# autonomousvision/LaRa

Hardware: AMD Instinct MI355X
Metric: novel-view frames/sec @512x512 (4-view in, 2DGS fwd+bwd) (higher is better)
Workload: dtype f32 raster + bf16-MFMA/f32-accumulate encoder (+ bf16-autocast coarse decoder MLP, as the reference's bf16-mixed)

## Files before the change

### lara_amd/csrc/composite.hip

```cpp
#include "common.h"
#include "wave.h"

namespace {

constexpr int FWD_CHUNK = 512;
constexpr int REC4 = 6;

__device__ __forceinline__ void cross3(const float a[3], const float b[3], float o[3]) {
    o[0] = a[1] * b[2] - a[2] * b[1];
    o[1] = a[2] * b[0] - a[0] * b[2];
    o[2] = a[0] * b[1] - a[1] * b[0];
}

template <int CHUNK>
__device__ __forceinline__ uint32_t stage_entry(const float4 *__restrict__ geom, const uint32_t id,
                                                const float4 cb, const bool valid, const float X0,
                                                const float Y0, float4 *rec, uint32_t *ids,
                                                const int e = threadIdx.x, uint2 *mask_out = nullptr) {
    float4 r0 = make_float4(0.f, 0.f, 0.f, 0.f), r1 = r0, r2 = r0, r3 = r0, r4 = r0, r5 = r0;
    uint32_t mask_lo = 0, mask_hi = 0, rectpack = 0;
    int gx0 = 0, gx1 = -1, gy0 = 0, gy1 = -1;
    if (valid) {
        gx0 = (int)ceilf(fminf(fmaxf((cb.x - X0 - 1.f) * 0.5f, 0.f), 8.f));
        gx1 = (int)floorf(fminf(fmaxf((cb.y - X0) * 0.5f, -1.f), 7.f));
        gy0 = (int)ceilf(fminf(fmaxf((cb.z - Y0 - 1.f) * 0.5f, 0.f), 8.f));
        gy1 = (int)floorf(fminf(fmaxf((cb.w - Y0) * 0.5f, -1.f), 7.f));
    }
    if (gx0 <= gx1 && gy0 <= gy1) {
        const float4 *g = geom + (size_t)id * 5;
        const float4 g0 = g[0], g1 = g[1], g2 = g[2], g3 = g[3], g4 = g[4];
        const float Tu[3] = {g0.x, g0.y, g0.z}, Tv[3] = {g0.w, g1.x, g1.y}, Tw[3] = {g1.z, g1.w, g2.x};
        const float k0[3] = {X0 * Tw[0] - Tu[0], X0 * Tw[1] - Tu[1], X0 * Tw[2] - Tu[2]};
        const float l0[3] = {Y0 * Tw[0] - Tv[0], Y0 * Tw[1] - Tv[1], Y0 * Tw[2] - Tv[2]};
        float A[3], B[3], C[3];
        cross3(k0, l0, A);
        cross3(Tw, l0, B);
        cross3(k0, Tw, C);
        const float cx = g2.y - X0, cy = g2.z - Y0, opa = g2.w;
        const float tau = 2.0f * __logf(255.0f * opa) * 1.001f + 0.01f;
        const float nb = B[0] * B[0] + B[1] * B[1], qa = nb - tau * B[2] * B[2];
        const bool ellipse = qa > 1e-5f * (nb + tau * B[2] * B[2]);
        const float inv_qa = ellipse ? __builtin_amdgcn_rcpf(qa) : 0.f;
        const float bx0 = (float)(2 * gx0), bx1 = (float)(2 * gx1 + 1);
        uint32_t colsum = 0;
        for (int by = gy0; by <= gy1; by++) {
            float lo = 1e9f, hi = -1e9f;
#pragma unroll
            for (int q = 0; q < 2; q++) {
                const float y = (float)(2 * by + q);
                const float u0 = A[0] + y * C[0], u1 = A[1] + y * C[1], u2 = A[2] + y * C[2];
                const float qb = u0 * B[0] + u1 * B[1] - tau * (u2 * B[2]);
                const float qc = u0 * u0 + u1 * u1 - tau * (u2 * u2);
                const float disc = qb * qb - qa * qc + 4e-6f * (qb * qb);
                if (!ellipse) {
                    lo = bx0; hi = bx1;
                } else if (disc >= 0.f) {
                    const float sq = __builtin_amdgcn_sqrtf(disc);
                    lo = fminf(lo, (-qb - sq) * inv_qa);
                    hi = fmaxf(hi, (-qb + sq) * inv_qa);
                }
                const float h = 0.5f * tau - (y - cy) * (y - cy);
                if (h >= 0.f) {
                    const float sh = __builtin_amdgcn_sqrtf(h);
                    lo = fminf(lo, cx - sh);
                    hi = fmaxf(hi, cx + sh);
                }
            }
            const int ilo = (int)ceilf(fmaxf(lo - 0.02f, bx0)), ihi = (int)floorf(fminf(hi + 0.02f, bx1));
            if (ilo <= ihi) {
                const uint32_t cols = ((2u << (ihi >> 1)) - 1u) & ~((1u << (ilo >> 1)) - 1u);
                colsum |= cols;
                if (by < 4) mask_lo |= cols << (8 * by);
                else mask_hi |= cols << (8 * (by - 4));
            }
        }
        if (colsum) {
            const int rx0 = __builtin_ctz(colsum), rx1 = 31 - __builtin_clz(colsum);
            const int ry0 = mask_lo ? (__builtin_ctz(mask_lo) >> 3) : 4 + (__builtin_ctz(mask_hi) >> 3);
            const int ry1 = mask_hi ? 4 + ((31 - __builtin_clz(mask_hi)) >> 3) : ((31 - __builtin_clz(mask_lo)) >> 3);
            rectpack = (uint32_t)rx0 | ((uint32_t)rx1 << 4) | ((uint32_t)ry0 << 8) | ((uint32_t)ry1 << 12) | (1u << 16);
            r0 = make_float4(A[0], A[1], A[2], B[0]);
            r1 = make_float4(B[1], B[2], C[0], C[1]);
            r2 = make_float4(C[2], cx, cy, Tw[0]);
            r3 = make_float4(Tw[1], Tw[2], opa, __uint_as_float(mask_lo));
            r4 = make_float4(g3.x, g3.y, g3.z, g4.x);
            r5 = make_float4(g4.y, g4.z, __uint_as_float(mask_hi), 0.f);
        }
    }
    rec[0 * CHUNK + e] = r0; rec[1 * CHUNK + e] = r1; rec[2 * CHUNK + e] = r2;
    rec[3 * CHUNK + e] = r3; rec[4 * CHUNK + e] = r4; rec[5 * CHUNK + e] = r5;
    if (ids) ids[e] = valid ? id : 0u;
    if (mask_out && valid) *mask_out = make_uint2(mask_lo, mask_hi);
    return rectpack;
}

template <int CHUNK>
__device__ __forceinline__ void stage_entry_masked(const float4 *__restrict__ geom, const uint32_t id, const uint2 mask,
                                                   const bool valid, const float X0, const float Y0, float4 *rec,
                                                   uint32_t *ids, const int e) {
    float4 r0 = make_float4(0.f, 0.f, 0.f, 0.f), r1 = r0, r2 = r0, r3 = r0, r4 = r0, r5 = r0;
    if (valid && (mask.x | mask.y)) {
        const float4 *g = geom + (size_t)id * 5;
        const float4 g0 = g[0], g1 = g[1], g2 = g[2], g3 = g[3], g4 = g[4];
        const float Tu[3] = {g0.x, g0.y, g0.z}, Tv[3] = {g0.w, g1.x, g1.y}, Tw[3] = {g1.z, g1.w, g2.x};
        const float k0[3] = {X0 * Tw[0] - Tu[0], X0 * Tw[1] - Tu[1], X0 * Tw[2] - Tu[2]};
        const float l0[3] = {Y0 * Tw[0] - Tv[0], Y0 * Tw[1] - Tv[1], Y0 * Tw[2] - Tv[2]};
        float A[3], B[3], C[3];
        cross3(k0, l0, A);
        cross3(Tw, l0, B);
        cross3(k0, Tw, C);
        r0 = make_float4(A[0], A[1], A[2], B[0]);
        r1 = make_float4(B[1], B[2], C[0], C[1]);
        r2 = make_float4(C[2], g2.y - X0, g2.z - Y0, Tw[0]);
        r3 = make_float4(Tw[1], Tw[2], g2.w, __uint_as_float(mask.x));
        r4 = make_float4(g3.x, g3.y, g3.z, g4.x);
        r5 = make_float4(g4.y, g4.z, __uint_as_float(mask.y), 0.f);
    }
    rec[0 * CHUNK + e] = r0; rec[1 * CHUNK + e] = r1; rec[2 * CHUNK + e] = r2;
    rec[3 * CHUNK + e] = r3; rec[4 * CHUNK + e] = r4; rec[5 * CHUNK + e] = r5;
    ids[e] = valid ? id : 0u;
}

struct Hit {
    float sx, sy, rz, depth, G, alpha, ddx, ddy;
    bool use3d;
};

struct EntryRec { float4 r0, r1, r2, r3; };
template <int CHUNK>
__device__ __forceinline__ EntryRec load_entry(const float4 *rec, const int j) {
    EntryRec e;
    e.r0 = rec[0 * CHUNK + j]; e.r1 = rec[1 * CHUNK + j]; e.r2 = rec[2 * CHUNK + j]; e.r3 = rec[3 * CHUNK + j];
    return e;
}

__device__ __forceinline__ bool eval_rec(const EntryRec &e, const float lx, const float ly, Hit &h,
                                         float Tw[3], float &opa) {
    const float4 r0 = e.r0, r1 = e.r1, r2 = e.r2, r3 = e.r3;
    const float px = r0.x + lx * r0.w + ly * r1.z;
    const float py = r0.y + lx * r1.x + ly * r1.w;
    const float pz = r0.z + lx * r1.y + ly * r2.x;
    Tw[0] = r2.w; Tw[1] = r3.x; Tw[2] = r3.y; opa = r3.z;
    h.rz = __builtin_amdgcn_rcpf(pz);
    h.sx = px * h.rz; h.sy = py * h.rz;
    const float rho3d = h.sx * h.sx + h.sy * h.sy;
    h.ddx = r2.y - lx; h.ddy = r2.z - ly;
    const float rho2d = FILTER_INV_SQUARE * (h.ddx * h.ddx + h.ddy * h.ddy);
    h.use3d = rho3d <= rho2d;
    const float rho = fminf(rho3d, rho2d);
    h.depth = h.use3d ? (h.sx * Tw[0] + h.sy * Tw[1]) + Tw[2] : Tw[2];
    const float power = -0.5f * rho;
    h.G = __expf(power);
    h.alpha = fminf(0.99f, opa * h.G);
    return (pz != 0.0f) & (h.depth >= NEAR_N) & !(power > 0.0f) & !(h.alpha < 1.0f / 255.0f);
}

__device__ __forceinline__ unsigned long long quad_masks(const uint32_t bm, const int qx4, const int grp) {
    unsigned long long m = 0ull;
#pragma unroll
    for (int g = 0; g < 16; g++) {
        const int bit = (g >> 2) * 8 + qx4 + (g & 3);
        const unsigned long long b = __ballot((bm >> bit) & 1u);
        m = (grp == g) ? b : m;
    }
    return m;
}

struct FwdPixel {
    float T = 1.0f, C0 = 0.f, C1 = 0.f, C2 = 0.f, N0 = 0.f, N1 = 0.f, N2 = 0.f;
    float Dd = 0.f, M1 = 0.f, M2 = 0.f, distortion = 0.f, median_depth = 0.f;
    uint32_t last_contributor = 0, median_contributor = 0;
    bool done = false;

    template <int CHUNK>
    __device__ __forceinline__ void blend(const float4 *rec, const int j, const int base, bool valid,
                                          const Hit &h) {
        valid = valid && !done;
        const float test_T = T * (1.0f - h.alpha);
        const bool kill = valid && test_T < 0.0001f;
        done = done || kill;
        valid = valid && !kill;
        if (__ballot(valid) == 0ull) return;
        const float4 r4 = rec[4 * CHUNK + j], r5 = rec[5 * CHUNK + j];
        const float a = valid ? h.alpha : 0.f;
        const float depth = valid ? h.depth : 1.0f;
        const float w = a * T;
        const float A = 1.0f - T;
        const float mm = FAR_N / (FAR_N - NEAR_N) * (1.0f - NEAR_N * __builtin_amdgcn_rcpf(depth));
        distortion += (mm * mm * A + M2 - 2.0f * mm * M1) * w;
        Dd += depth * w;
        M1 += mm * w;
        M2 += mm * mm * w;
        const bool med = valid && T > 0.5f;
        median_depth = med ? depth : median_depth;
        median_contributor = med ? (uint32_t)(base + j + 1) : median_contributor;
        N0 += r4.x * w; N1 += r4.y * w; N2 += r4.z * w;
        C0 += r4.w * w; C1 += r5.x * w; C2 += r5.y * w;
        T = valid ? test_T : T;
        last_contributor = valid ? (uint32_t)(base + j + 1) : last_contributor;
    }

};

template <bool KEEP>
__global__ void __launch_bounds__(256)
composite_fwd_kernel(ViewDev v, const uint32_t *__restrict__ header, const uint2 *__restrict__ ranges,
                     const uint32_t *__restrict__ point_list, const float4 *__restrict__ geom,
                     const uint32_t *__restrict__ tile_order, const float4 *__restrict__ cullbox,
                     float *__restrict__ final_T, uint32_t *__restrict__ n_contrib,
                     const uint32_t *__restrict__ seg_base, const uint32_t *__restrict__ seg_cnt,
                     float *__restrict__ ckpt, uint2 *__restrict__ pair_mask, uint32_t *__restrict__ tile_maxc,
                     uint32_t *__restrict__ seg_cost,
                     float *__restrict__ out_color, float *__restrict__ out_allmap, const ViewBatch vb) {
    {
        const long long sst = vb.state_stride, HWb = (long long)v.H * v.W * 4;
        header = l2d_view_ptr(header, sst); ranges = l2d_view_ptr(ranges, sst); point_list = l2d_view_ptr(point_list, sst);
        geom = l2d_view_ptr(geom, sst); tile_order = l2d_view_ptr(tile_order, sst); cullbox = l2d_view_ptr(cullbox, sst);
        final_T = l2d_view_ptr(final_T, sst); n_contrib = l2d_view_ptr(n_contrib, sst); seg_base = l2d_view_ptr(seg_base, sst);
        seg_cnt = l2d_view_ptr(seg_cnt, sst); ckpt = l2d_view_ptr(ckpt, sst); pair_mask = l2d_view_ptr(pair_mask, sst);
        tile_maxc = l2d_view_ptr(tile_maxc, sst); seg_cost = l2d_view_ptr(seg_cost, sst);
        out_color = l2d_view_ptr(out_color, 3 * HWb); out_allmap = l2d_view_ptr(out_allmap, 7 * HWb);
        v.bg = vb.bg[blockIdx.z];
    }
    constexpr int CHUNK = FWD_CHUNK;
    static_assert(L2D_SEG % FWD_CHUNK == 0, "segment boundaries must fall on round boundaries");
    __shared__ float4 rec[REC4 * CHUNK];
    __shared__ unsigned long long qmask[4][16][CHUNK / 64];
    uint32_t &s_cost = *(uint32_t *)&rec[5 * CHUNK + 0].w;
    uint32_t &s_tmax = *(uint32_t *)&rec[5 * CHUNK + 1].w;
    uint32_t &s_ndone = *(uint32_t *)&rec[5 * CHUNK + 2].w;
    const int tile = (v.dbg & 8u) ? (int)blockIdx.x : (int)tile_order[blockIdx.x];
    const int tx = tile % v.gx, ty = tile / v.gx;
    const int wave = threadIdx.x >> 6, lane = threadIdx.x & 63;
    const int grp = lane >> 2;
    const int lxi = (wave & 1) * 8 + (grp & 3) * 2 + (lane & 1);
    const int lyi = (wave >> 1) * 8 + (grp >> 2) * 2 + ((lane >> 1) & 1);
    const int pxi = tx * TILE + lxi, pyi = ty * TILE + lyi;
    const bool inside = pxi < v.W && pyi < v.H;
    const size_t HW = (size_t)v.H * v.W;
    const size_t pix = (size_t)pyi * v.W + pxi;
    const float lx = (float)lxi, ly = (float)lyi;
    const float X0 = (float)(tx * TILE), Y0 = (float)(ty * TILE);

    if (header[1]) {
        if (inside) {
            const float qnan = __uint_as_float(0x7fc00000u);
            for (int ch = 0; ch < 3; ch++) out_color[ch * HW + pix] = qnan;
            for (int ch = 0; ch < 7; ch++) out_allmap[ch * HW + pix] = qnan;
            if (KEEP) {
                for (int ch = 0; ch < L2D_CKPT_F; ch++) final_T[pix + ch * HW] = qnan;
                n_contrib[pix] = 0; n_contrib[pix + HW] = 0;
            }
        }
        return;
    }

    const uint2 range = ranges[tile];
    const int total = (int)(range.y - range.x);
    const int lo = 0, hi = total;
    FwdPixel px;
    px.done = !inside;
    uint32_t *dbg_hdr = const_cast<uint32_t *>(header);
    const long long dbg_t0 = (v.dbg & 32u) ? (long long)__builtin_readcyclecounter() : 0ll;
    int dbg_rounds = 0;

    const int tid = threadIdx.x;
    const uint32_t cost_nb = KEEP ? seg_cnt[tile] : 0u;
    uint32_t *const cost_full = KEEP ? seg_cost + seg_base[tile] : nullptr,
             *const cost_last = KEEP ? seg_cost + (v.cap / L2D_SEG + 1u) + tile : nullptr;
    if (KEEP)
        for (uint32_t q = tid; q <= cost_nb; q += 256) *(q < cost_nb ? cost_full + q : cost_last) = 0u;
    int cost_round = -1;
    constexpr int SPT = CHUNK / 256;
    uint32_t id1[SPT], id2[SPT];
    float4 cb1[SPT];
#pragma unroll
    for (int q = 0; q < SPT; q++) {
        const int o = lo + q * 256 + tid;
        id1[q] = o < hi ? point_list[range.x + o] : 0u;
        id2[q] = CHUNK + o < hi ? point_list[range.x + CHUNK + o] : 0u;
    }
#pragma unroll
    for (int q = 0; q < SPT; q++) cb1[q] = lo + q * 256 + tid < hi ? cullbox[id1[q]] : make_float4(0.f, 0.f, 0.f, 0.f);
    if (threadIdx.x < 3) *(uint32_t *)&rec[5 * CHUNK + threadIdx.x].w = 0u;
    __syncthreads();
    for (int base = lo; base < hi; base += CHUNK) {
        {
            const bool wave_done = __ballot(px.done) == ~0ull;
            if (wave_done && lane == 0) atomicAdd(&s_ndone, 1u);
            __syncthreads();
            if (s_ndone == 4u) break;
        }
        if (KEEP && tid == 0) {
            if (cost_round >= 0) { if ((uint32_t)cost_round < cost_nb) cost_full[cost_round] = s_cost; else *cost_last += s_cost; }
            s_cost = 0u;
        }
        cost_round = (base - lo) / CHUNK;
        dbg_rounds++;
        if (KEEP && base && base % L2D_SEG == 0 && !px.done) {
            float *ck = ckpt + ((size_t)seg_base[tile] + (size_t)(base / L2D_SEG - 1)) * (L2D_CKPT_F * 256) + tid;
            ck[0 * 256] = px.T; ck[1 * 256] = px.M1; ck[2 * 256] = px.M2;
            ck[3 * 256] = px.C0; ck[4 * 256] = px.C1; ck[5 * 256] = px.C2;
            ck[6 * 256] = px.Dd; ck[7 * 256] = px.N0; ck[8 * 256] = px.N1; ck[9 * 256] = px.N2;
        }
#pragma unroll
        for (int q = 0; q < SPT; q++) {
            const int o = q * 256 + tid;
            const uint32_t id0 = id1[q];
            const float4 cb0 = cb1[q];
            id1[q] = id2[q];
            id2[q] = base + 2 * CHUNK + o < hi ? point_list[range.x + base + 2 * CHUNK + o] : 0u;
            cb1[q] = base + CHUNK + o < hi ? cullbox[id1[q]] : make_float4(0.f, 0.f, 0.f, 0.f);
            stage_entry<CHUNK>(geom, id0, cb0, base + o < hi, X0, Y0, rec, nullptr, o,
                               KEEP && base + o < hi ? pair_mask + range.x + base + o : nullptr);
        }
        __syncthreads();
        if (__ballot(!px.done) == 0ull) continue;
        const int nw = (min(CHUNK, hi - base) + 63) >> 6;
        unsigned long long *qm = &qmask[wave][grp][0];
#pragma unroll 1
        for (int w = 0; w < nw; w++) {
            const float4 *mrec = rec + ((wave >> 1) ? 5 : 3) * CHUNK + w * 64 + lane;
            const uint32_t bm = __float_as_uint((wave >> 1) ? mrec->z : mrec->w);
            unsigned long long m = 0ull;
            if (__ballot((bm & (0x0f0f0f0fu << ((wave & 1) * 4))) != 0u) != 0ull) m = quad_masks(bm, (wave & 1) * 4, grp);
            if ((lane & 3) == 0) qm[w] = m;
        }
        int w = 0;
        unsigned long long mm = qm[0];
        if (((__ballot(px.done) >> (lane & ~3)) & 0xfull) == 0xfull) { mm = 0ull; w = nw; }
        auto next = [&](bool &has, int &j) {
            while (mm == 0ull && w + 1 < nw) { w++; mm = qm[w]; }
            has = mm != 0ull;
            j = has ? 64 * w + __builtin_ctzll(mm) : 0;
            mm &= mm - 1ull;
        };
        bool hA0, hA1, hB0 = false, hB1 = false;
        int jA0, jA1, jB0 = 0, jB1 = 0;
        next(hA0, jA0);
        next(hA1, jA1);
        EntryRec rA0 = load_entry<CHUNK>(rec, jA0), rA1 = load_entry<CHUNK>(rec, jA1), rB0, rB1;
        auto trip = [&](const EntryRec &c0, const EntryRec &c1, const int j0, const int j1, const bool has0, const bool has1,
                        EntryRec &x0, EntryRec &x1, int &k0, int &k1, bool &n0, bool &n1) {
            next(n0, k0);
            next(n1, k1);
            x0 = load_entry<CHUNK>(rec, k0);
            x1 = load_entry<CHUNK>(rec, k1);
            Hit h0, h1;
            float Tw0[3], Tw1[3], opa0, opa1;
            const bool e0 = eval_rec(c0, lx, ly, h0, Tw0, opa0) && has0;
            const bool e1 = eval_rec(c1, lx, ly, h1, Tw1, opa1) && has1;
            if (v.dbg & 4u) {
                atomicAdd(&dbg_hdr[4], ((lane & 3) == 0) ? (unsigned)has0 + (unsigned)has1 : 0u);
                atomicAdd(&dbg_hdr[5], (unsigned)e0 + (unsigned)e1);
                if (lane == 0) atomicAdd(&dbg_hdr[6], 1u);
            }
            px.blend<CHUNK>(rec, j0, base, e0, h0);
            px.blend<CHUNK>(rec, j1, base, e1, h1);
            if (((__ballot(px.done) >> (lane & ~3)) & 0xfull) == 0xfull) { mm = 0ull; w = nw; n0 = false; n1 = false; }
        };
        uint32_t ntrips = 0;
        while (true) {
            if (__ballot(hA0) == 0ull) break;
            trip(rA0, rA1, jA0, jA1, hA0, hA1, rB0, rB1, jB0, jB1, hB0, hB1);
            ntrips++;
            if (__ballot(hB0) == 0ull) break;
            trip(rB0, rB1, jB0, jB1, hB0, hB1, rA0, rA1, jA0, jA1, hA0, hA1);
            ntrips++;
        }
        if (KEEP && lane == 0 && ntrips) atomicAdd(&s_cost, ntrips);
    }
    const float T = px.T;
    if (KEEP) {
        if (threadIdx.x == 0) s_tmax = 0u;
        __syncthreads();
        uint32_t m = px.last_contributor;
#pragma unroll
        for (int d = 1; d < 64; d <<= 1) m = max(m, (uint32_t)__shfl_xor((int)m, d, 64));
        if (lane == 0) atomicMax(&s_tmax, m);
        __syncthreads();
        if (threadIdx.x == 0) {
            tile_maxc[tile] = s_tmax;
            if (cost_round >= 0) { if ((uint32_t)cost_round < cost_nb) cost_full[cost_round] = s_cost; else *cost_last += s_cost; }
        }
    }
// ... 49 lines not shown
#pragma unroll
    for (int c = 0; c < 3; c++) {
        float d = dp[c];
        asm volatile("" : "+v"(d));
        const float t = d + dpp_move<0xB1, 0xf>(d);
        const float tq = q[c] + dpp_move<0xB1, 0xf>(q[c]);
        const float mine = k.a1 * t + (k.a2 * d + k.a3 * tq);
        const float send = k.b1 * t + (k.b2 * d + k.b3 * tq);
        r[c] = mine + dpp_move<0x4E, 0xf>(send);
    }
    float v1[5];
#pragma unroll
    for (int i = 0; i < 5; i++) {
        const float mine = b0 ? h[2 * i + 1] : h[2 * i];
        const float send = b0 ? h[2 * i] : h[2 * i + 1];
        v1[i] = mine + dpp_move<0xB1, 0xf>(send);
    }
#pragma unroll
    for (int i = 0; i < 2; i++) {
        const float mine = b1 ? v1[2 * i + 1] : v1[2 * i];
        const float send = b1 ? v1[2 * i] : v1[2 * i + 1];
        r[3 + i] = mine + dpp_move<0x4E, 0xf>(send);
    }
    r[5] = v1[4] + dpp_move<0x4E, 0xf>(v1[4]);
}
__device__ __forceinline__ void quad_reduce_scatter16(const float dp[3], const float q[3], const float h[4], const QuadCoef &k,
                                                      float r[4], const int lane) {
    const bool b0 = lane & 1, b1 = lane & 2;
#pragma unroll
    for (int c = 0; c < 3; c++) {
        float d = dp[c], qq = q[c];
        asm volatile("" : "+v"(d));
        asm volatile("" : "+v"(qq));
        const float t = d + dpp_move<0xB1, 0xf>(d);
        const float tq = qq + dpp_move<0xB1, 0xf>(qq);
        const float mine = k.a1 * t + (k.a2 * d + k.a3 * tq);
        const float send = k.b1 * t + (k.b2 * d + k.b3 * tq);
        r[c] = mine + dpp_move<0x4E, 0xf>(send);
    }
    float v1[2];
#pragma unroll
    for (int i = 0; i < 2; i++) {
        const float mine = b0 ? h[2 * i + 1] : h[2 * i];
        const float send = b0 ? h[2 * i] : h[2 * i + 1];
        v1[i] = mine + dpp_move<0xB1, 0xf>(send);
    }
    const float mine = b1 ? v1[1] : v1[0];
    const float send = b1 ? v1[0] : v1[1];
    r[3] = mine + dpp_move<0x4E, 0xf>(send);
}

constexpr int SLAB_WIN = 128;
constexpr int SLAB_CHUNK = 128;
constexpr int SLAB_POOL = 374;
constexpr int SLAB_F = 24;
constexpr int SLAB_F_COLOR = 16;
constexpr int SLAB_POOL_COLOR = SLAB_POOL * SLAB_F / SLAB_F_COLOR;

template <bool MAPS>
__global__ void __launch_bounds__(256)
composite_bwd_kernel(ViewDev v, const uint32_t *__restrict__ header, const uint2 *__restrict__ ranges,
                     const uint32_t *__restrict__ point_list, const float4 *__restrict__ geom,
                     const uint32_t *__restrict__ tile_order, const float4 *__restrict__ cullbox,
                     const float *__restrict__ final_T, const uint32_t *__restrict__ n_contrib,
                     const uint32_t *__restrict__ seg_base, const uint32_t *__restrict__ seg_cnt,
                     const uint32_t *__restrict__ bwd_order,
                     const uint2 *__restrict__ bwd_items, const float *__restrict__ ckpt,
                     const uint2 *__restrict__ pair_mask, const uint32_t *__restrict__ tile_maxc,
                     const float *__restrict__ dL_dcolor, const float *__restrict__ dL_dallmap,
                     const uint32_t *__restrict__ pair_pos,
                     float4 *__restrict__ pair_grad, uint8_t *__restrict__ pair_valid, const ViewBatch vb) {
    {
        const long long sst = vb.state_stride, qst = vb.scratch_stride, HWb = (long long)v.H * v.W * 4;
        header = l2d_view_ptr(header, sst); ranges = l2d_view_ptr(ranges, sst); point_list = l2d_view_ptr(point_list, sst);
        geom = l2d_view_ptr(geom, sst); tile_order = l2d_view_ptr(tile_order, sst); cullbox = l2d_view_ptr(cullbox, sst);
        final_T = l2d_view_ptr(final_T, sst); n_contrib = l2d_view_ptr(n_contrib, sst); seg_base = l2d_view_ptr(seg_base, sst);
        seg_cnt = l2d_view_ptr(seg_cnt, sst); bwd_order = l2d_view_ptr(bwd_order, sst); bwd_items = l2d_view_ptr(bwd_items, sst);
        ckpt = l2d_view_ptr(ckpt, sst); pair_mask = l2d_view_ptr(pair_mask, sst); pair_pos = l2d_view_ptr(pair_pos, sst);
        tile_maxc = l2d_view_ptr(tile_maxc, sst);
        pair_grad = l2d_view_ptr(pair_grad, qst); pair_valid = l2d_view_ptr(pair_valid, qst);
        dL_dcolor = l2d_view_ptr(dL_dcolor, 3 * HWb); dL_dallmap = l2d_view_ptr(dL_dallmap, 7 * HWb);
        v.bg = vb.bg[blockIdx.z];
    }
    constexpr int WIN = SLAB_WIN;
    constexpr int POOL = MAPS ? SLAB_POOL : SLAB_POOL_COLOR, SF = MAPS ? SLAB_F : SLAB_F_COLOR;
    __shared__ float4 rec[REC4 * WIN];
    __shared__ __attribute__((aligned(16))) float pool[(POOL + 1) * SF];
    __shared__ uint16_t s_base_[2][SLAB_CHUNK];
    __shared__ unsigned long long s_live_[2][SLAB_CHUNK];
    __shared__ uint32_t s_ql[64];
    __shared__ uint32_t s_id_[2][WIN];
    __shared__ uint2 s_mask[WIN];
    __shared__ int s_nfit_[2];
    __shared__ uint32_t s_total_[2];
    if (header[1]) return;
    const unsigned long long dbg_t0 = (v.dbg & 32u) ? wall_clock64() : 0ull;
    int dbg_rounds = 0;
    uint32_t dbg_windows = 0, dbg_trips = 0, dbg_entries = 0, dbg_slots = 0, dbg_rows = 0;
    unsigned long long dbg_tp = 0ull;
    uint32_t dbg_ph[5] = {0u, 0u, 0u, 0u, 0u};
#define DBG_PHASE(k) do { if (v.dbg & 64u) { const unsigned long long t__ = __builtin_readcyclecounter(); dbg_ph[k] += (uint32_t)(t__ - dbg_tp); dbg_tp = t__; } } while (0)
    if (v.dbg & 64u) dbg_tp = __builtin_readcyclecounter();
    const uint32_t n_full = header[3];
    int tile, seg;
    if (header[22]) {
        if (blockIdx.x >= n_full + (uint32_t)v.tiles) return;
        const uint2 it = bwd_items[blockIdx.x];
        tile = (int)it.x; seg = (int)it.y;
    } else if (blockIdx.x < n_full) {
        const uint2 it = bwd_items[blockIdx.x];
        tile = (int)it.x; seg = (int)it.y;
    } else if (blockIdx.x - n_full < (uint32_t)v.tiles) {
        tile = (int)bwd_order[blockIdx.x - n_full];
        seg = (int)seg_cnt[tile];
    } else {
        return;
    }
    const uint2 range = ranges[tile];
    const int seg_lo = seg * L2D_SEG;
    const int seg_hi = seg == (int)seg_cnt[tile] ? (int)(range.y - range.x) : seg_lo + L2D_SEG;
    const int total = min((int)tile_maxc[tile], seg_hi);
    const int lo = seg_lo;
    if (total <= lo) return;
    const int tx = tile % v.gx, ty = tile / v.gx;
    const int tid = threadIdx.x, wave = tid >> 6, lane = tid & 63;
    const int grp = lane >> 2;
    const int lxi = (wave & 1) * 8 + (grp & 3) * 2 + (lane & 1);
    const int lyi = (wave >> 1) * 8 + (grp >> 2) * 2 + ((lane >> 1) & 1);
    const int pxi = tx * TILE + lxi, pyi = ty * TILE + lyi;
    const bool inside = pxi < v.W && pyi < v.H;
    const size_t HW = (size_t)v.H * v.W;
    const size_t pix = inside ? (size_t)pyi * v.W + pxi : 0;
    const float lx = (float)lxi, ly = (float)lyi;
    const float X0 = (float)(tx * TILE), Y0 = (float)(ty * TILE);

    const float T_final = inside ? final_T[pix] : 0.f;
    float T = T_final;
    const uint32_t last_contributor = inside ? n_contrib[pix] : 0u;
    const uint32_t median_contributor = (MAPS && inside) ? n_contrib[pix + HW] : 0u;
    float dpix[3] = {0.f, 0.f, 0.f}, dnrm[3] = {0.f, 0.f, 0.f};
    float dL_ddepth = 0.f, dL_daccum = 0.f, dL_dmedian = 0.f, dL_dreg = 0.f;
    float final_D = 0.f, final_D2 = 0.f;
    if (inside) {
        for (int ch = 0; ch < 3; ch++) dpix[ch] = dL_dcolor[ch * HW + pix];
        if constexpr (MAPS) {
            dL_ddepth = dL_dallmap[0 * HW + pix];
            dL_daccum = dL_dallmap[1 * HW + pix];
// ... 58 lines not shown
                    volatile unsigned long long *vlive = live_;
                    vlive[2 * lane] = 0ull;
                    vlive[2 * lane + 1] = 0ull;
                    if (jm < SLAB_CHUNK) atomicOr(&live_[jm], 1ull << lane);
                    __builtin_amdgcn_wave_barrier();
                    la = vlive[2 * lane];
                    lb = la | vlive[2 * lane + 1];
                    unsigned long long ex = lb;
#pragma unroll
                    for (int d = 1; d < 64; d <<= 1) {
                        const uint32_t ylo = __shfl_up((uint32_t)ex, d, 64), yhi = __shfl_up((uint32_t)(ex >> 32), d, 64);
                        if (lane >= d) ex |= ((unsigned long long)yhi << 32) | ylo;
                    }
                    const uint32_t plo = __shfl_up((uint32_t)ex, 1, 64), phi = __shfl_up((uint32_t)(ex >> 32), 1, 64);
                    const unsigned long long before = lane ? (((unsigned long long)phi << 32) | plo) : 0ull;
                    la |= before; lb |= before;
                }
                uint32_t c[2];
#pragma unroll
                for (int q = 0; q < 2; q++) {
                    const int slot = s0_ + 2 * lane + q;
                    unsigned long long mk = 0ull;
                    if (slot < wcnt_) {
                        const uint2 mw = side ? s_mask[slot] : make_uint2(__float_as_uint(rec[3 * WIN + slot].w), __float_as_uint(rec[5 * WIN + slot].z));
                        mk = (((unsigned long long)mw.y << 32) | mw.x) & (q ? lb : la);
                    }
                    live_[2 * lane + q] = mk;
                    c[q] = (uint32_t)__builtin_popcountll(mk);
                }
                uint32_t incl = c[0] + c[1];
#pragma unroll
                for (int d = 1; d < 64; d <<= 1) {
                    const uint32_t y = __shfl_up(incl, d, 64);
                    if (lane >= d) incl += y;
                }
                const uint32_t b0 = incl - c[0] - c[1], b1 = incl - c[1];
                const unsigned long long f0 = __ballot(s0_ + 2 * lane < wcnt_ && b1 <= (uint32_t)POOL);
                const unsigned long long f1 = __ballot(s0_ + 2 * lane + 1 < wcnt_ && incl <= (uint32_t)POOL);
                const int L = f1 == ~0ull ? 64 : __builtin_ctzll(~f1);
                if (lane == 0) s_nfit_[buf] = L == 64 ? 128 : 2 * L + (int)((f0 >> L) & 1ull);
                base_[2 * lane] = (uint16_t)b0;
                base_[2 * lane + 1] = (uint16_t)b1;
                if (lane == 63) s_total_[buf] = incl;
    };
    {
        const int wcnt = min(WIN, total - lo);
        if (stager) {
            const uint32_t id0 = total - 1 - se >= lo ? point_list[range.x + total - 1 - se] : 0u;
            const uint2 mk0 = total - 1 - se >= lo ? pair_mask[range.x + total - 1 - se] : make_uint2(0u, 0u);
            id1 = total - WIN - 1 - se >= lo ? point_list[range.x + total - WIN - 1 - se] : 0u;
            mk1 = total - WIN - 1 - se >= lo ? pair_mask[range.x + total - WIN - 1 - se] : make_uint2(0u, 0u);
            id2 = total - 2 * WIN - 1 - se >= lo ? point_list[range.x + total - 2 * WIN - 1 - se] : 0u;
            mk2 = total - 2 * WIN - 1 - se >= lo ? pair_mask[range.x + total - 2 * WIN - 1 - se] : make_uint2(0u, 0u);
            stage_entry_masked<WIN>(geom, id0, mk0, se < wcnt, X0, Y0, rec, s_id_[0], se);
        }
        __syncthreads();
        if (wave == 3) size_round(total, wcnt, 0, 0, false);
        __syncthreads();
        DBG_PHASE(0);
    }
    int cur = 0, wb = 0;
    for (int whi = total; whi > lo; whi -= WIN) {
        const int wcnt = min(WIN, whi - lo);
        const bool more_windows = whi - WIN > lo;
        dbg_windows++;
        if (stager) s_mask[se] = mk1;
        unsigned long long wm0 = 0ull, wm1 = 0ull;

        for (int s0 = 0; s0 < wcnt;) {
            dbg_rounds++;
            const unsigned long long *const s_live = s_live_[cur];
            const uint16_t *const s_base = s_base_[cur];
            const uint32_t *const s_id = s_id_[wb];
            const int nfit = s_nfit_[cur];
            if (v.dbg & 512u) { dbg_entries += (uint32_t)nfit; dbg_slots += nfit < SLAB_CHUNK ? (uint32_t)s_base[nfit] : min(s_total_[cur], (uint32_t)POOL); }

            {
                if (s0 == 0) {
#pragma unroll
                    for (int k = 0; k < 2; k++) {
                        const float4 *mrec = rec + ((wave >> 1) ? 5 : 3) * WIN + 64 * k + lane;
                        const uint32_t bm = __float_as_uint((wave >> 1) ? mrec->z : mrec->w);
                        unsigned long long m = 0ull;
                        if (__ballot((bm & (0x0f0f0f0fu << ((wave & 1) * 4))) != 0u) != 0ull) m = quad_masks(bm, (wave & 1) * 4, grp);
                        if (k == 0) wm0 = m; else wm1 = m;
                    }
                }
                unsigned long long m0 = wm0, m1 = wm1;
                {
                    int sh = s0;
                    if (sh >= 64) { m0 = m1; m1 = 0ull; sh -= 64; }
                    if (sh) { m0 = (m0 >> sh) | (m1 << (64 - sh)); m1 >>= sh; }
                    if (nfit < 64) { m0 &= (1ull << nfit) - 1ull; m1 = 0ull; }
                    else if (nfit < 128) m1 &= (1ull << (nfit - 64)) - 1ull;
                }
                const int jmin = whi - s0 - (int)quad_last;
                if (jmin > 0) {
                    m0 = jmin >= 64 ? 0ull : m0 & (~0ull << jmin);
                    m1 = jmin >= 128 ? 0ull : (jmin > 64 ? m1 & (~0ull << (jmin - 64)) : m1);
                }
                uint32_t mm = (uint32_t)m0, q1 = (uint32_t)(m0 >> 32), q2 = (uint32_t)m1, q3 = (uint32_t)(m1 >> 32);
                int jb = 0;
                auto trip = [&]() __attribute__((always_inline)) {
                    dbg_trips++;
                    while (mm == 0u && (q1 | q2 | q3) != 0u) { mm = q1; q1 = q2; q2 = q3; q3 = 0u; jb += 32; }
                    const bool has = mm != 0u;
                    const int j = jb + (has ? __builtin_ctz(mm) : 0);
                    mm &= mm - 1u;
                    const int ws = s0 + j;
                    const uint32_t contributor = (uint32_t)(whi - 1 - ws);
                    const EntryRec ent = load_entry<WIN>(rec, ws);
                    Hit h;
                    float Tw[3], opa;
                    const bool active = eval_rec(ent, lx, ly, h, Tw, opa) && has && contributor < last_contributor;
                    const float4 r4 = rec[4 * WIN + ws], r5 = rec[5 * WIN + ws];
                    const float nrm[3] = {r4.x, r4.y, r4.z}, rgb[3] = {r4.w, r5.x, r5.y};
                    if constexpr (!MAPS) {
                        (void)nrm;
                        const float alpha = active ? h.alpha : 0.f;
                        const float inv_1ma = __builtin_amdgcn_rcpf(1.f - alpha);
                        const float T_new = T * inv_1ma;
                        const float w = alpha * T_new;
                        const float gval = __builtin_fmaf(rgb[2], dpix[2], __builtin_fmaf(rgb[0], dpix[0], rgb[1] * dpix[1]));
                        const float accum_new = mul_legacy(last_alpha, last_g) + (1.f - last_alpha) * accum_g;
                        float dL_dalpha = gval - accum_new;
                        dL_dalpha = __builtin_fmaf(T_new, dL_dalpha, -((T_final * inv_1ma) * bg_dot_dpixel));
                        T = T_new;
                        accum_g = accum_new;
                        last_g = gval;
                        last_alpha = alpha;
                        const float da = active ? dL_dalpha : 0.f;
                        const float sx = h.sx, sy = h.sy;
                        const float rz3 = (active && h.use3d) ? h.rz : 0.f;
                        const float qG = opa * da * h.G;
                        const float dL_dsx = -mul_legacy(qG, sx), dL_dsy = -mul_legacy(qG, sy);
                        const float dpx = dL_dsx * rz3, dpy = dL_dsy * rz3;
                        const float dpv[3] = {dpx, dpy, -(mul_legacy(dpx, sx) + mul_legacy(dpy, sy))};
                        const float qG2 = h.use3d ? 0.f : -FILTER_INV_SQUARE * qG;
                        const float q3[3] = {h.G * da, qG2 * h.ddx, qG2 * h.ddy};
                        const float h4[4] = {w * dpix[0], w * dpix[1], w * dpix[2], w};
// ... 23 lines not shown
                    const float dL_dweight = (final_D2 + m_d * m_d * final_A - 2.f * m_d * final_D) * dL_dreg;
                    dL_dalpha += dL_dweight - last_dL_dT;
                    const float dLdT_new = mul_legacy(alpha, dL_dweight) + (1.f - alpha) * last_dL_dT;
                    const float dL_dmd = 2.0f * (T_new * alpha) * (m_d * final_A - final_D) * dL_dreg;
                    dL_dz += dL_dmd * dmd_dd;
                    dL_dalpha *= T_new;
                    dL_dalpha += (-T_final * inv_1ma) * bg_dot_dpixel;
                    dL_dz += w * dL_ddepth;
                    T = T_new;
                    accum_g = accum_new;
                    last_g = gval;
                    last_alpha = alpha;
                    last_dL_dT = dLdT_new;
                    const float ww = w, da = active ? dL_dalpha : 0.f, dz = active ? dL_dz : 0.f;
                    const float sx = h.sx, sy = h.sy;
                    const float rz3 = (active && h.use3d) ? h.rz : 0.f;
                    const float qv[3] = {mul_legacy(dz, sx), mul_legacy(dz, sy), dz};
                    const float qG = opa * da * h.G;
                    const float dL_dsx = dz * Tw[0] - mul_legacy(qG, sx);
                    const float dL_dsy = dz * Tw[1] - mul_legacy(qG, sy);
                    const float dpx = dL_dsx * rz3, dpy = dL_dsy * rz3;
                    const float dpv[3] = {dpx, dpy, -(mul_legacy(dpx, sx) + mul_legacy(dpy, sy))};
                    const float qG2 = h.use3d ? 0.f : -FILTER_INV_SQUARE * qG;
                    const float hv[10] = {qG2 * h.ddx, qG2 * h.ddy, ww * dnrm[0], ww * dnrm[1], ww * dnrm[2], h.G * da,
                                          ww * dpix[0], ww * dpix[1], ww * dpix[2], ww};
                    float r[6];
                    quad_reduce_scatter(dpv, qv, hv, qcoef, r, lane);
#pragma unroll
                    for (int i = 0; i < 6; i++) asm volatile("" : "+v"(r[i]));
                    const unsigned long long lv = s_live[has ? j : 0];
                    const int rank = __builtin_popcount((uint32_t)lv & below_lo) + __builtin_popcount((uint32_t)(lv >> 32) & below_hi);
                    float *ps = pool + ((int)s_base[has ? j : 0] + rank) * SLAB_F + (lane & 3);
                    if (has) {
                        ps[0] = r[0]; ps[4] = r[1]; ps[8] = r[2]; ps[12] = r[3]; ps[16] = r[4];
                        if (!(lane & 2)) ps[20] = r[5];
                    }
                    }
                };
                while (__ballot((mm | q1 | q2 | q3) != 0u) != 0ull) {
                    trip();
                    if (__ballot((mm | q1 | q2 | q3) != 0u) == 0ull) break;
                    trip();
                }
            }
            __syncthreads();
            DBG_PHASE(3);

            if ((wave << 5) < nfit && !(v.dbg & 2u)) {
                const int e = tid >> 1, part = tid & 1;
                const int ws = min(s0 + e, WIN - 1);
                const bool has = e < nfit;
                const int cnt = has ? __builtin_popcountll(s_live[e]) : 0;
                float4 gq0 = make_float4(0.f, 0.f, 0.f, 0.f), gq1 = gq0, gq2 = gq0;
                if (cnt && part == 0) {
                    const float4 *gm = geom + (size_t)s_id[ws] * 5;
                    gq0 = gm[0]; gq1 = gm[1]; gq2 = gm[2];
                }
                constexpr int NG = MAPS ? 22 : 16;
                float g[NG];
                const float4 *ps = (const float4 *)(pool + (int)s_base[e] * SF);
                {
                    const float4 *p0 = part < cnt ? ps + part * (SF / 4) : (const float4 *)(pool + POOL * SF);
#pragma unroll
                    for (int q = 0; q < NG / 4; q++) {
                        const float4 t = p0[q];
                        g[4 * q] = t.x; g[4 * q + 1] = t.y; g[4 * q + 2] = t.z; g[4 * q + 3] = t.w;
                    }
                    if constexpr (MAPS) {
                        const float2 t2 = *(const float2 *)(p0 + 5);
                        g[20] = t2.x; g[21] = t2.y;
                    }
                }
                for (int i = part + 2; i < cnt; i += 2) {
#pragma unroll
                    for (int q = 0; q < NG / 4; q++) {
                        const float4 t = ps[i * (SF / 4) + q];
                        g[4 * q] += t.x; g[4 * q + 1] += t.y; g[4 * q + 2] += t.z; g[4 * q + 3] += t.w;
                    }
                    if constexpr (MAPS) {
                        const float2 t2 = *(const float2 *)(ps + i * (SF / 4) + 5);
                        g[20] += t2.x; g[21] += t2.y;
                    }
                }
#pragma unroll
                for (int k = 0; k < NG; k++) g[k] += dpp_move<0xB1, 0xf>(g[k]);
                const bool touched = (MAPS ? g[21] : g[15]) > 0.f;
                if (part == 0 && touched) {
                    const uint32_t p = range.x + (uint32_t)(whi - 1 - ws);
                    const float4 g0 = gq0, g1 = gq1, g2 = gq2;
                    const float Tu[3] = {g0.x, g0.y, g0.z}, Tv[3] = {g0.w, g1.x, g1.y}, Tw[3] = {g1.z, g1.w, g2.x};
                    const float k0[3] = {X0 * Tw[0] - Tu[0], X0 * Tw[1] - Tu[1], X0 * Tw[2] - Tu[2]};
                    const float l0[3] = {Y0 * Tw[0] - Tv[0], Y0 * Tw[1] - Tv[1], Y0 * Tw[2] - Tv[2]};
                    const float a[3] = {g[0], MAPS ? g[4] : g[1], MAPS ? g[8] : g[2]};
                    const float b[3] = {MAPS ? g[1] : g[4], g[5], MAPS ? g[9] : g[6]};
                    const float cc[3] = {MAPS ? g[2] : g[8], MAPS ? g[6] : g[9], g[10]};
                    const float qd[3] = {MAPS ? g[3] : 0.f, MAPS ? g[7] : 0.f, MAPS ? g[11] : 0.f};
                    float t1[3], t2[3], dk0[3], dl0[3], dTw[3];
                    cross3(l0, a, t1); cross3(Tw, cc, t2);
                    for (int i = 0; i < 3; i++) dk0[i] = t1[i] + t2[i];
                    cross3(a, k0, t1); cross3(b, Tw, t2);
                    for (int i = 0; i < 3; i++) dl0[i] = t1[i] + t2[i];
                    cross3(l0, b, t1); cross3(cc, k0, t2);
                    for (int i = 0; i < 3; i++) {
                        dTw[i] = t1[i] + t2[i] + X0 * dk0[i] + Y0 * dl0[i];
                        if constexpr (MAPS) dTw[i] += qd[i];
                    }
                    const uint32_t q = pair_pos[p];
                    float4 *row = pair_grad + (size_t)q * (GRAD_F / 4);
                    row[0] = make_float4(-dk0[0], -dk0[1], -dk0[2], -dl0[0]);
                    row[1] = make_float4(-dl0[1], -dl0[2], dTw[0], dTw[1]);
                    if constexpr (MAPS) {
                        row[2] = make_float4(dTw[2], g[12], g[13], g[14]);
                        row[3] = make_float4(g[15], g[16], g[17], g[18]);
                        row[4] = make_float4(g[19], g[20], 0.f, 0.f);
                    } else {
                        row[2] = make_float4(dTw[2], g[13], g[14], 0.f);
                        row[3] = make_float4(0.f, 0.f, g[12], g[3]);
                        row[4] = make_float4(g[7], g[11], 0.f, 0.f);
                    }
                    pair_valid[q] = 1;
                    dbg_rows++;
                }
            }
            const bool last_round = s0 + nfit >= wcnt;
            if (stager && last_round && more_windows) {
                stage_entry_masked<WIN>(geom, id1, mk1, se < min(WIN, whi - WIN - lo), X0, Y0, rec, s_id_[wb ^ 1], se);
                id1 = id2;
                mk1 = mk2;
                id2 = whi - 3 * WIN - 1 - se >= lo ? point_list[range.x + whi - 3 * WIN - 1 - se] : 0u;
                mk2 = whi - 3 * WIN - 1 - se >= lo ? pair_mask[range.x + whi - 3 * WIN - 1 - se] : make_uint2(0u, 0u);
            }
            if (wave == 3) {
                if (!last_round) size_round(whi, wcnt, s0 + nfit, cur ^ 1, false);
                else if (more_windows) size_round(whi - WIN, min(WIN, whi - WIN - lo), 0, cur ^ 1, true);
            }
            __syncthreads();
            DBG_PHASE(4);
            s0 += nfit;
            cur ^= 1;
        }
        wb ^= 1;
    }
    if ((v.dbg & 64u) && tid == 0) {
        DBG_PHASE(4);
        uint32_t *h = const_cast<uint32_t *>(header);
        for (int k = 0; k < 5; k++) atomicAdd(&h[16 + k], dbg_ph[k] >> 6);
    }
    if (v.dbg & 512u) {
        uint32_t *h = const_cast<uint32_t *>(header);
        if (tid == 0) {
            atomicAdd(&h[24], 1u); atomicAdd(&h[25], dbg_windows); atomicAdd(&h[26], (uint32_t)dbg_rounds);
            atomicAdd(&h[28], dbg_entries); atomicAdd(&h[29], dbg_slots);
        }
        if (lane == 0) atomicAdd(&h[27], dbg_trips);
        if (dbg_rows) atomicAdd(&h[30], dbg_rows);
    }
    if ((v.dbg & 32u) && tid == 0) {
        uint32_t *h = const_cast<uint32_t *>(header);
        const unsigned long long t1 = wall_clock64();
        atomicMax(&h[8], (uint32_t)(t1 - dbg_t0));
        atomicMax((unsigned long long *)&h[12], ((unsigned long long)(uint32_t)(t1 - dbg_t0) << 32) |
                                                    ((unsigned long long)dbg_rounds << 16) | (unsigned long long)blockIdx.x);
        atomicAdd(&h[9], (uint32_t)(t1 - dbg_t0));
        atomicMax(&h[10], ~(uint32_t)dbg_t0);
        atomicMax(&h[11], (uint32_t)t1);
    }
}

__global__ void __launch_bounds__(64)
selftest_butterfly_kernel(const float *__restrict__ in, float *__restrict__ out) {
    const int lane = threadIdx.x, q4 = lane & 3, grp = lane >> 2;
    const float lx = (float)((grp & 3) * 2 + (lane & 1)), ly = (float)((grp >> 2) * 2 + ((lane >> 1) & 1));
    float dp[3], q[3], h[10], r[6];
    for (int k = 0; k < 3; k++) { dp[k] = in[lane * 16 + k]; q[k] = in[lane * 16 + 3 + k]; }
    for (int k = 0; k < 10; k++) h[k] = in[lane * 16 + 6 + k];
    quad_reduce_scatter(dp, q, h, quad_coef(lane, lx, ly), r, lane);
    float *dst = out + (lane >> 2) * 24 + q4;
    for (int i = 0; i < 5; i++) dst[4 * i] = r[i];
    if (q4 < 2) dst[20] = r[5];
// ... 103 lines not shown
```

Measured before the change: 923.6.

## Build per-quad entry masks via wave bit-transpose at staging time

Replaces the per-wave 16-ballot quad_masks construction with a 64x64 bit transpose (shuffles, DPP and alignbit) done once per entry when it is staged, storing the resulting per-2x2-block words in shared memory indexed by block. Forward and backward consumers then read their block's word directly instead of rebuilding masks each chunk. The backward kernel also issues the pair_pos load early, alongside the geometry loads, so its latency is hidden, and SLAB_POOL shrinks to make room for the new LDS array within the three-workgroups-per-CU budget. The trade-off is a smaller pool and extra transpose work for every staged entry.

```diff
diff --git a/lara_amd/csrc/composite.hip b/lara_amd/csrc/composite.hip
--- a/lara_amd/csrc/composite.hip
+++ b/lara_amd/csrc/composite.hip
@@ -12,11 +12,55 @@
     o[2] = a[0] * b[1] - a[1] * b[0];
 }
 
+__device__ __forceinline__ uint32_t rot_merge(const uint32_t own, const uint32_t got, const uint32_t keep, const uint32_t rot) {
+    return (own & keep) | (__builtin_amdgcn_alignbit(got, got, rot) & ~keep);
+}
+__device__ __forceinline__ unsigned long long bit_transpose64(uint32_t lo, uint32_t hi, int lane) {
+    asm volatile("" : "+v"(lane));
+    {
+        const bool up = lane & 32;
+        const uint32_t got = (uint32_t)__shfl_xor((int)(up ? lo : hi), 32, 64);
+        lo = up ? got : lo;
+        hi = up ? hi : got;
+    }
+#define L2D_TR_STEP(J, M, XCH)                                                                  \
+    {                                                                                           \
+        const bool up = lane & J;                                                               \
+        const uint32_t keep = up ? M : ~M, rot = up ? J : 32 - J;                               \
+        const uint32_t glo = XCH(lo), ghi = XCH(hi);                                            \
+        lo = rot_merge(lo, glo, keep, rot);                                                     \
+        hi = rot_merge(hi, ghi, keep, rot);                                                     \
+    }
+#define L2D_XCH_SHFL16(x) (uint32_t)__shfl_xor((int)(x), 16, 64)
+#define L2D_XCH_ROR8(x) (uint32_t)__builtin_amdgcn_update_dpp(0, (int)(x), 0x128, 0xf, 0xf, false)
+#define L2D_XCH_SHFL4(x) (uint32_t)__shfl_xor((int)(x), 4, 64)
+#define L2D_XCH_QUAD2(x) (uint32_t)__builtin_amdgcn_update_dpp(0, (int)(x), 0x4E, 0xf, 0xf, false)
+#define L2D_XCH_QUAD1(x) (uint32_t)__builtin_amdgcn_update_dpp(0, (int)(x), 0xB1, 0xf, 0xf, false)
+    L2D_TR_STEP(16, 0xffff0000u, L2D_XCH_SHFL16)
+    L2D_TR_STEP(8, 0xff00ff00u, L2D_XCH_ROR8)
+    L2D_TR_STEP(4, 0xf0f0f0f0u, L2D_XCH_SHFL4)
+    L2D_TR_STEP(2, 0xccccccccu, L2D_XCH_QUAD2)
+    L2D_TR_STEP(1, 0xaaaaaaaau, L2D_XCH_QUAD1)
+#undef L2D_TR_STEP
+#undef L2D_XCH_SHFL16
+#undef L2D_XCH_ROR8
+#undef L2D_XCH_SHFL4
+#undef L2D_XCH_QUAD2
+#undef L2D_XCH_QUAD1
+    return ((unsigned long long)hi << 32) | lo;
+}
+__device__ __forceinline__ void file_entries(unsigned long long *words, const uint32_t mask_lo, const uint32_t mask_hi, const int lane) {
+    unsigned long long w = 0ull;
+    if (__ballot((mask_lo | mask_hi) != 0u) != 0ull) w = bit_transpose64(mask_lo, mask_hi, lane);
+    words[lane] = w;
+}
+
 template <int CHUNK>
 __device__ __forceinline__ uint32_t stage_entry(const float4 *__restrict__ geom, const uint32_t id,
                                                 const float4 cb, const bool valid, const float X0,
                                                 const float Y0, float4 *rec, uint32_t *ids,
-                                                const int e = threadIdx.x, uint2 *mask_out = nullptr) {
+                                                unsigned long long *qwords, const int e = threadIdx.x,
+                                                uint2 *mask_out = nullptr) {
     float4 r0 = make_float4(0.f, 0.f, 0.f, 0.f), r1 = r0, r2 = r0, r3 = r0, r4 = r0, r5 = r0;
     uint32_t mask_lo = 0, mask_hi = 0, rectpack = 0;
     int gx0 = 0, gx1 = -1, gy0 = 0, gy1 = -1;
@@ -91,13 +135,14 @@
     rec[3 * CHUNK + e] = r3; rec[4 * CHUNK + e] = r4; rec[5 * CHUNK + e] = r5;
     if (ids) ids[e] = valid ? id : 0u;
     if (mask_out && valid) *mask_out = make_uint2(mask_lo, mask_hi);
+    file_entries(qwords + (e >> 6) * 64, mask_lo, mask_hi, e & 63);
     return rectpack;
 }
 
 template <int CHUNK>
 __device__ __forceinline__ void stage_entry_masked(const float4 *__restrict__ geom, const uint32_t id, const uint2 mask,
                                                    const bool valid, const float X0, const float Y0, float4 *rec,
-                                                   uint32_t *ids, const int e) {
+                                                   uint32_t *ids, unsigned long long *qwords, const int e) {
     float4 r0 = make_float4(0.f, 0.f, 0.f, 0.f), r1 = r0, r2 = r0, r3 = r0, r4 = r0, r5 = r0;
     if (valid && (mask.x | mask.y)) {
         const float4 *g = geom + (size_t)id * 5;
@@ -119,6 +164,7 @@
     rec[0 * CHUNK + e] = r0; rec[1 * CHUNK + e] = r1; rec[2 * CHUNK + e] = r2;
     rec[3 * CHUNK + e] = r3; rec[4 * CHUNK + e] = r4; rec[5 * CHUNK + e] = r5;
     ids[e] = valid ? id : 0u;
+    file_entries(qwords + (e >> 6) * 64, valid ? mask.x : 0u, valid ? mask.y : 0u, e & 63);
 }
 
 struct Hit {
@@ -153,17 +199,6 @@
     h.G = __expf(power);
     h.alpha = fminf(0.99f, opa * h.G);
     return (pz != 0.0f) & (h.depth >= NEAR_N) & !(power > 0.0f) & !(h.alpha < 1.0f / 255.0f);
-}
-
-__device__ __forceinline__ unsigned long long quad_masks(const uint32_t bm, const int qx4, const int grp) {
-    unsigned long long m = 0ull;
-#pragma unroll
-    for (int g = 0; g < 16; g++) {
-        const int bit = (g >> 2) * 8 + qx4 + (g & 3);
-        const unsigned long long b = __ballot((bm >> bit) & 1u);
-        m = (grp == g) ? b : m;
-    }
-    return m;
 }
 
 struct FwdPixel {
@@ -225,7 +260,7 @@
     constexpr int CHUNK = FWD_CHUNK;
     static_assert(L2D_SEG % FWD_CHUNK == 0, "segment boundaries must fall on round boundaries");
     __shared__ float4 rec[REC4 * CHUNK];
-    __shared__ unsigned long long qmask[4][16][CHUNK / 64];
+    __shared__ unsigned long long qmask[CHUNK / 64][64];
     uint32_t &s_cost = *(uint32_t *)&rec[5 * CHUNK + 0].w;
     uint32_t &s_tmax = *(uint32_t *)&rec[5 * CHUNK + 1].w;
     uint32_t &s_ndone = *(uint32_t *)&rec[5 * CHUNK + 2].w;
@@ -311,26 +346,18 @@
             id1[q] = id2[q];
             id2[q] = base + 2 * CHUNK + o < hi ? point_list[range.x + base + 2 * CHUNK + o] : 0u;
             cb1[q] = base + CHUNK + o < hi ? cullbox[id1[q]] : make_float4(0.f, 0.f, 0.f, 0.f);
-            stage_entry<CHUNK>(geom, id0, cb0, base + o < hi, X0, Y0, rec, nullptr, o,
+            stage_entry<CHUNK>(geom, id0, cb0, base + o < hi, X0, Y0, rec, nullptr, &qmask[0][0], o,
                                KEEP && base + o < hi ? pair_mask + range.x + base + o : nullptr);
         }
         __syncthreads();
         if (__ballot(!px.done) == 0ull) continue;
         const int nw = (min(CHUNK, hi - base) + 63) >> 6;
-        unsigned long long *qm = &qmask[wave][grp][0];
-#pragma unroll 1
-        for (int w = 0; w < nw; w++) {
-            const float4 *mrec = rec + ((wave >> 1) ? 5 : 3) * CHUNK + w * 64 + lane;
-            const uint32_t bm = __float_as_uint((wave >> 1) ? mrec->z : mrec->w);
-            unsigned long long m = 0ull;
-            if (__ballot((bm & (0x0f0f0f0fu << ((wave & 1) * 4))) != 0u) != 0ull) m = quad_masks(bm, (wave & 1) * 4, grp);
-            if ((lane & 3) == 0) qm[w] = m;
-        }
+        const unsigned long long *qm = &qmask[0][(lyi >> 1) * 8 + (lxi >> 1)];
         int w = 0;
         unsigned long long mm = qm[0];
         if (((__ballot(px.done) >> (lane & ~3)) & 0xfull) == 0xfull) { mm = 0ull; w = nw; }
         auto next = [&](bool &has, int &j) {
-            while (mm == 0ull && w + 1 < nw) { w++; mm = qm[w]; }
+            while (mm == 0ull && w + 1 < nw) { w++; mm = qm[64 * w]; }
             has = mm != 0ull;
             j = has ? 64 * w + __builtin_ctzll(mm) : 0;
             mm &= mm - 1ull;
@@ -486,7 +513,7 @@
 
 constexpr int SLAB_WIN = 128;
 constexpr int SLAB_CHUNK = 128;
-constexpr int SLAB_POOL = 374;
+constexpr int SLAB_POOL = 364;
 constexpr int SLAB_F = 24;
 constexpr int SLAB_F_COLOR = 16;
 constexpr int SLAB_POOL_COLOR = SLAB_POOL * SLAB_F / SLAB_F_COLOR;
@@ -527,6 +554,9 @@
     __shared__ uint2 s_mask[WIN];
     __shared__ int s_nfit_[2];
     __shared__ uint32_t s_total_[2];
+    __shared__ unsigned long long s_qw[WIN / 64][64];
+    static_assert(sizeof(rec) + sizeof(pool) + sizeof(s_base_) + sizeof(s_live_) + sizeof(s_ql) + sizeof(s_id_) + sizeof(s_mask) +
+                  sizeof(s_qw) + sizeof(s_nfit_) + sizeof(s_total_) <= 53248, "three workgroups per CU need <= 53 248 bytes of LDS");
     if (header[1]) return;
     const unsigned long long dbg_t0 = (v.dbg & 32u) ? wall_clock64() : 0ull;
     int dbg_rounds = 0;
@@ -691,7 +721,7 @@
             mk1 = total - WIN - 1 - se >= lo ? pair_mask[range.x + total - WIN - 1 - se] : make_uint2(0u, 0u);
             id2 = total - 2 * WIN - 1 - se >= lo ? point_list[range.x + total - 2 * WIN - 1 - se] : 0u;
             mk2 = total - 2 * WIN - 1 - se >= lo ? pair_mask[range.x + total - 2 * WIN - 1 - se] : make_uint2(0u, 0u);
-            stage_entry_masked<WIN>(geom, id0, mk0, se < wcnt, X0, Y0, rec, s_id_[0], se);
+            stage_entry_masked<WIN>(geom, id0, mk0, se < wcnt, X0, Y0, rec, s_id_[0], &s_qw[0][0], se);
         }
         __syncthreads();
         if (wave == 3) size_round(total, wcnt, 0, 0, false);
@@ -715,16 +745,7 @@
             if (v.dbg & 512u) { dbg_entries += (uint32_t)nfit; dbg_slots += nfit < SLAB_CHUNK ? (uint32_t)s_base[nfit] : min(s_total_[cur], (uint32_t)POOL); }
 
             {
-                if (s0 == 0) {
-#pragma unroll
-                    for (int k = 0; k < 2; k++) {
-                        const float4 *mrec = rec + ((wave >> 1) ? 5 : 3) * WIN + 64 * k + lane;
-                        const uint32_t bm = __float_as_uint((wave >> 1) ? mrec->z : mrec->w);
-                        unsigned long long m = 0ull;
-                        if (__ballot((bm & (0x0f0f0f0fu << ((wave & 1) * 4))) != 0u) != 0ull) m = quad_masks(bm, (wave & 1) * 4, grp);
-                        if (k == 0) wm0 = m; else wm1 = m;
-                    }
-                }
+                if (s0 == 0) { wm0 = s_qw[0][my_blk]; wm1 = s_qw[1][my_blk]; }
                 unsigned long long m0 = wm0, m1 = wm1;
                 {
                     int sh = s0;
@@ -854,9 +875,11 @@
                 const bool has = e < nfit;
                 const int cnt = has ? __builtin_popcountll(s_live[e]) : 0;
                 float4 gq0 = make_float4(0.f, 0.f, 0.f, 0.f), gq1 = gq0, gq2 = gq0;
+                uint32_t row_pos = 0u;
                 if (cnt && part == 0) {
                     const float4 *gm = geom + (size_t)s_id[ws] * 5;
                     gq0 = gm[0]; gq1 = gm[1]; gq2 = gm[2];
+                    row_pos = pair_pos[range.x + (uint32_t)(whi - 1 - ws)];
                 }
                 constexpr int NG = MAPS ? 22 : 16;
                 float g[NG];
@@ -888,7 +911,6 @@
                 for (int k = 0; k < NG; k++) g[k] += dpp_move<0xB1, 0xf>(g[k]);
                 const bool touched = (MAPS ? g[21] : g[15]) > 0.f;
                 if (part == 0 && touched) {
-                    const uint32_t p = range.x + (uint32_t)(whi - 1 - ws);
                     const float4 g0 = gq0, g1 = gq1, g2 = gq2;
                     const float Tu[3] = {g0.x, g0.y, g0.z}, Tv[3] = {g0.w, g1.x, g1.y}, Tw[3] = {g1.z, g1.w, g2.x};
                     const float k0[3] = {X0 * Tw[0] - Tu[0], X0 * Tw[1] - Tu[1], X0 * Tw[2] - Tu[2]};
@@ -907,7 +929,7 @@
                         dTw[i] = t1[i] + t2[i] + X0 * dk0[i] + Y0 * dl0[i];
                         if constexpr (MAPS) dTw[i] += qd[i];
                     }
-                    const uint32_t q = pair_pos[p];
+                    const uint32_t q = row_pos;
                     float4 *row = pair_grad + (size_t)q * (GRAD_F / 4);
                     row[0] = make_float4(-dk0[0], -dk0[1], -dk0[2], -dl0[0]);
                     row[1] = make_float4(-dl0[1], -dl0[2], dTw[0], dTw[1]);
@@ -926,7 +948,7 @@
             }
             const bool last_round = s0 + nfit >= wcnt;
             if (stager && last_round && more_windows) {
-                stage_entry_masked<WIN>(geom, id1, mk1, se < min(WIN, whi - WIN - lo), X0, Y0, rec, s_id_[wb ^ 1], se);
+                stage_entry_masked<WIN>(geom, id1, mk1, se < min(WIN, whi - WIN - lo), X0, Y0, rec, s_id_[wb ^ 1], &s_qw[0][0], se);
                 id1 = id2;
                 mk1 = mk2;
                 id2 = whi - 3 * WIN - 1 - se >= lo ? point_list[range.x + whi - 3 * WIN - 1 - se] : 0u;
```

Result: faster. 932.9 (median of 6 runs) (+1.0%).
